# sdwyc/ROLO

Measured on AMD Instinct MI355X. Metric: scans/sec (128k-pt frame, 20 GN iters), higher is better.
Workload: dtype f64

## Files before the change

rolo_amd/csrc/knn_cov.hip:

```cpp
#include <cstdio>
#include <cstring>
#include <string.h>
#include "rolo_internal.hpp"
#include "switches.hpp"
#include "dev_math.hpp"
#include "voxel_dev.hpp"
#ifdef ROLO_KNN_ROCPRIM_SORT
#include <rocprim/rocprim.hpp>
#endif
#include <cfloat>
#include <climits>

namespace rolo {

namespace {


constexpr int BBOX_BLOCKS = 128;
constexpr int BBOX_PART = 16;

__global__ __launch_bounds__(256) void bbox_kernel(KnnPair A, int* bbox) {
  __shared__ float smn[4][3], smx[4][3];
  const int which = blockIdx.x / BBOX_BLOCKS, blk = blockIdx.x - which * BBOX_BLOCKS;
  const float4* __restrict__ p = A.c[which].xyz;
// ... 512 lines not shown
bool knn_voxel_fuse_supported() {
#ifdef ROLO_KNN_ROCPRIM_SORT
  return false;
#else
  return true;
#endif
}

size_t knn_bbox_ints() { return BBOX_PART + 2 * BBOX_BLOCKS * 6; }

size_t knn_sort_temp_bytes(int n) {
#ifdef ROLO_KNN_ROCPRIM_SORT
  size_t bytes = 0;
  (void)rocprim::radix_sort_pairs(nullptr, bytes, (uint32_t*)nullptr, (uint32_t*)nullptr, (uint32_t*)nullptr, (uint32_t*)nullptr,
                                  (size_t)n, 0, 31, (hipStream_t)0);
  return bytes;
#else
  (void)n;
  return sizeof(int) * SORT_PASSES * SORT_NB * SORT_D;
#endif
}

hipError_t launch_knn_build(const KnnPair& A_in, void* sort_tmp, size_t sort_tmp_bytes, uint32_t* keys0, uint32_t* keys1,
                            uint32_t* vals0, uint32_t* vals1, int* bbox, const VoxelFuse& vf, hipStream_t s) {
  KnnPair A = A_in;
  bool have_parts = true;
  for (int i = 0; i < A.n_clouds; i++) have_parts = have_parts && A.c[i].bpart != nullptr && A.c[i].n_bpart > 0;
  if (!have_parts) for (int i = 0; i < A.n_clouds; i++) { A.c[i].bpart = bbox + BBOX_PART + i * BBOX_BLOCKS * 6; A.c[i].n_bpart = BBOX_BLOCKS; }
  const int nc = A.n_clouds;
  const int n_total = A.c[0].n + (nc > 1 ? A.c[1].n : 0);
#ifdef ROLO_KNN_ROCPRIM_SORT
  const int tile_ = ((n_total + SORT_NB - 1) / SORT_NB + SORT_T - 1) / SORT_T * SORT_T;
  if (!have_parts) bbox_kernel<<<BBOX_BLOCKS * nc, 256, 0, s>>>(A, bbox);
  morton_kernel<<<SORT_NB + (vf.enabled ? VF_CLEAR_BLOCKS : 0), SORT_T, 0, s>>>(A, bbox, keys0, vals0, n_total, tile_, nullptr, vf);
  hipError_t e = rocprim::radix_sort_pairs(sort_tmp, sort_tmp_bytes, keys0, keys1, vals0, vals1, (size_t)n_total, 0, nc > 1 ? KEY_BITS : KEY_BITS - 1, s);
  if (e != hipSuccess) return e;
  const uint32_t* order = vals1;
#else
  (void)sort_tmp_bytes;
  int* cnt = static_cast<int*>(sort_tmp);
  const int gvf = vf.enabled ? ((vf.n_tgt + SORT_PASSES - 1) / SORT_PASSES + SORT_T - 1) / SORT_T : 0;
  const int tile = ((n_total + SORT_NB - 1) / SORT_NB + SORT_T - 1) / SORT_T * SORT_T;
  if (!have_parts) bbox_kernel<<<BBOX_BLOCKS * nc, 256, 0, s>>>(A, bbox);
  morton_kernel<<<SORT_NB + (vf.enabled ? VF_CLEAR_BLOCKS : 0), SORT_T, 0, s>>>(A, bbox, keys0, vals0, n_total, tile, cnt, vf);
  uint32_t *ki = keys0, *vi = vals0, *ko = keys1, *vo = vals1;
  for (int p = 0; p < SORT_PASSES; p++) {
    if (p > 0) sort_hist_kernel<<<SORT_NB, SORT_T, 0, s>>>(ki, n_total, tile, p, cnt);
    sort_scatter_kernel<<<SORT_NB + gvf, SORT_T, 0, s>>>(ki, vi, ko, vo, n_total, tile, p, cnt, vf);
    uint32_t* t1 = ki; ki = ko; ko = t1; t1 = vi; vi = vo; vo = t1;
  }
  const uint32_t* order = vi;
#endif
  static_assert(256 % KNN_LEAF == 0 && (KNN_LEAF & (KNN_LEAF - 1)) == 0, "leaf_kernel reduces a leaf inside a wavefront");
  const int l0 = (A.c[0].P * KNN_LEAF + 255) / 256, l1 = nc > 1 ? (A.c[1].P * KNN_LEAF + 255) / 256 : 0;
  leaf_kernel<<<l0 + l1, 256, 0, s>>>(A, l0, order);
  constexpr int LPB = 256 / KNN_LEAF;
  int count0 = A.c[0].P >= LPB ? A.c[0].P / LPB : A.c[0].P, count1 = nc > 1 ? (A.c[1].P >= LPB ? A.c[1].P / LPB : A.c[1].P) : 1;
  while (count0 > 1 || count1 > 1) {
    const int chunk0 = count0 < 512 ? count0 : 512, chunk1 = count1 < 512 ? count1 : 512;
    const int b0 = count0 > 1 ? count0 / chunk0 : 0, b1 = count1 > 1 ? count1 / chunk1 : 0;
    tree_reduce_kernel<<<b0 + b1, 256, 0, s>>>(A.c[0].boxes, count0, chunk0, b0, nc > 1 ? A.c[1].boxes : nullptr, count1, chunk1);
    if (count0 > 1) count0 /= chunk0;
    if (count1 > 1) count1 /= chunk1;
  }
  return hipGetLastError();
}

#ifdef ROLO_KNN_STATS
extern "C" int rolo_debug_wave_records(unsigned* out ) {
  (void)hipDeviceSynchronize();
  return hipMemcpyFromSymbol(out, HIP_SYMBOL(g_knn_wave_rec), sizeof(unsigned) * 16384 * 8) == hipSuccess ? 0 : -1;
}
#endif

static inline int slice_blocks(const KnnCloud& c) { return (c.q_end - c.q_begin + 255) / 256; }

constexpr int KNN_SUB_MAX_PACKETS = 1792;
hipError_t launch_knn_walk(const KnnPair& A, int k, hipStream_t s, int* lanes_out, bool device_busy, bool moments) {
  if (lanes_out) *lanes_out = 1;
  constexpr int QPB = 256;
  const int n0 = A.c[0].q_end - A.c[0].q_begin, n1 = A.n_clouds > 1 ? A.c[1].q_end - A.c[1].q_begin : 0;
  const int g0 = (n0 + QPB - 1) / QPB, g1 = (n1 + QPB - 1) / QPB;
  if (g0 + g1 == 0) return hipSuccess;
  if (k > 64) {
    KnnPair R = A;
    for (int r = 0; 64 * r < k; r++) {
      const int kr = k - 64 * r < 64 ? k - 64 * r : 64;
      for (int i = 0; i < R.n_clouds; i++) { R.c[i].slot0 = 64 * r; R.c[i].k_total = k; }
      if (r == 0) knn_walk_kernel<64><<<g0 + g1, 256, 0, s>>>(R, g0, kr);
      else knn_walk_kernel<64, true><<<g0 + g1, 256, 0, s>>>(R, g0, kr);
    }
    return hipGetLastError();
  }
  if (k == 20) {
    const int sub_env = switches().knn_sub;
    const int packets = (n0 + 63) / 64 + (n1 + 63) / 64;
    const int lanes = sub_env < 0 ? (packets <= KNN_SUB_MAX_PACKETS ? 4 : (device_busy ? 0 : 2)) : (sub_env == 2 ? 2 : (sub_env ? 4 : 0));
    if (lanes_out) *lanes_out = lanes ? lanes : 1;
    if (lanes == 4) { const int s0 = (n0 + 63) / 64, s1 = (n1 + 63) / 64; if (moments) knn_walk_sub_kernel<4, true><<<s0 + s1, 256, 0, s>>>(A, s0); else knn_walk_sub_kernel<4><<<s0 + s1, 256, 0, s>>>(A, s0); }
    else if (lanes == 2) { const int s0 = (n0 + 127) / 128, s1 = (n1 + 127) / 128; if (moments) knn_walk_sub_kernel<2, true><<<s0 + s1, 256, 0, s>>>(A, s0); else knn_walk_sub_kernel<2><<<s0 + s1, 256, 0, s>>>(A, s0); }
    else if (moments) knn_walk_kernel<20, false, true><<<g0 + g1, 256, 0, s>>>(A, g0, k);
    else knn_walk_kernel<20><<<g0 + g1, 256, 0, s>>>(A, g0, k);
  }
  else if (k > 32) knn_walk_kernel<64><<<g0 + g1, 256, 0, s>>>(A, g0, k);
  else knn_walk_kernel<32><<<g0 + g1, 256, 0, s>>>(A, g0, k);
  return hipGetLastError();
}

hipError_t launch_knn_unstage(const KnnPair& A, bool own_slice_only, const VoxelFuse& vf, hipStream_t s) {
  const int g0 = own_slice_only ? slice_blocks(A.c[0]) : (A.c[0].n_sorted + 255) / 256;
  const int g1 = A.n_clouds > 1 ? (own_slice_only ? slice_blocks(A.c[1]) : (A.c[1].n_sorted + 255) / 256) : 0;
  if (g0 + g1 == 0) return hipSuccess;
  VoxelFuse v = vf;
  if (own_slice_only) v.enabled = 0;
  knn_unstage_kernel<<<g0 + g1, 256, 0, s>>>(A, g0, own_slice_only ? 1 : 0, v);
  return hipGetLastError();
}

hipError_t launch_knn_tail(const KnnPair& A, int k, int regularization, const VoxelFuse& vf, hipStream_t s, bool moments) {
  const int g0 = slice_blocks(A.c[0]), g1 = A.n_clouds > 1 ? slice_blocks(A.c[1]) : 0;
  if (g0 + g1 == 0) return hipSuccess;
  if (k > 64) knn_tail_loop_kernel<<<g0 + g1, 256, 0, s>>>(A, g0, k, regularization, vf);
  else if (k == 20 && moments) knn_tail_kernel<20, true><<<g0 + g1, 256, 0, s>>>(A, g0, k, regularization, vf);
  else if (k == 20) knn_tail_kernel<20><<<g0 + g1, 256, 0, s>>>(A, g0, k, regularization, vf);
  else if (k <= 32) knn_tail_kernel<32><<<g0 + g1, 256, 0, s>>>(A, g0, k, regularization, vf);
  else knn_tail_kernel<64><<<g0 + g1, 256, 0, s>>>(A, g0, k, regularization, vf);
  return hipGetLastError();
}

}
```

rolo_amd/csrc/knn_packet.hpp:

```cpp
#pragma once
#include "rolo_internal.hpp"
#include "dev_math.hpp"
#include "knn_seed_net.hpp"
#include <cfloat>
#include <climits>

#ifndef KNN_STAT
#ifdef ROLO_KNN_STATS
#define KNN_STAT(x) x
#else
#define KNN_STAT(x)
#endif
#endif

namespace rolo {
namespace {

constexpr int WALK_STACK = KNN_WALK_STACK;

ROLO_DEV float box_d2(const float4& lo, const float4& hi, const float4& q) {
  float dx = fmaxf(fmaxf(__fsub_rn(lo.x, q.x), __fsub_rn(q.x, hi.x)), 0.f);
  float dy = fmaxf(fmaxf(__fsub_rn(lo.y, q.y), __fsub_rn(q.y, hi.y)), 0.f);
  float dz = fmaxf(fmaxf(__fsub_rn(lo.z, q.z), __fsub_rn(q.z, hi.z)), 0.f);
  return __fadd_rn(__fadd_rn(__fmul_rn(dx, dx), __fmul_rn(dy, dy)), __fmul_rn(dz, dz));
}

ROLO_DEV double key_pack(float d2, int idx) {
  return __longlong_as_double((long long)(((unsigned long long)__float_as_uint(d2) << 32) | (unsigned)idx));
}
ROLO_DEV float key_d2(double k) { return __uint_as_float((unsigned)((unsigned long long)__double_as_longlong(k) >> 32)); }
ROLO_DEV int key_idx(double k) { return (int)(unsigned)((unsigned long long)__double_as_longlong(k) & 0xffffffffull); }

ROLO_DEV double vmin_f64(double a, double b) { double r; asm("v_min_f64 %0, %1, %2" : "=v"(r) : "v"(a), "v"(b)); return r; }
ROLO_DEV double vmax_f64(double a, double b) { double r; asm("v_max_f64 %0, %1, %2" : "=v"(r) : "v"(a), "v"(b)); return r; }
#ifndef ROLO_KNN_SPLIT_MINMAX
ROLO_DEV void insert_slot(double& ks, double ksm1, double c) { asm("v_min_f64 %0, %1, %0\n\tv_max_f64 %0, %2, %0" : "+&v"(ks) : "v"(c), "v"(ksm1)); }
#else
ROLO_DEV void insert_slot(double& ks, double ksm1, double c) { ks = vmax_f64(ksm1, vmin_f64(c, ks)); }
#endif
#ifndef ROLO_KNN_B1
#define ROLO_KNN_B1 15
#define ROLO_KNN_B2 10
#define ROLO_KNN_B3 5
#endif
template <int KMAX>
ROLO_DEV void insert_tiered(double (&K)[KMAX], double ck) {
  constexpr int B1 = KMAX == 20 ? ROLO_KNN_B1 : 3 * (KMAX / 4), B2 = KMAX == 20 ? ROLO_KNN_B2 : 2 * (KMAX / 4), B3 = KMAX == 20 ? ROLO_KNN_B3 : KMAX / 4;
#pragma unroll
  for (int s = KMAX - 1; s >= B1; s--) insert_slot(K[s], K[s - 1], ck);
  if (__any(ck < K[B1 - 1])) {
#pragma unroll
    for (int s = B1 - 1; s >= B2; s--) insert_slot(K[s], K[s - 1], ck);
    if (__any(ck < K[B2 - 1])) {
#pragma unroll
      for (int s = B2 - 1; s >= B3; s--) insert_slot(K[s], K[s - 1], ck);
      if (__any(ck < K[B3 - 1])) {
#pragma unroll
        for (int s = B3 - 1; s >= 1; s--) insert_slot(K[s], K[s - 1], ck);
        K[0] = vmin_f64(ck, K[0]);
      }
    }
  }
}

ROLO_DEV void sload_leaf(const float4* __restrict__ p, float4 (&pts)[KNN_LEAF]) {
#pragma unroll
  for (int u = 0; u < KNN_LEAF; u++) pts[u] = p[u];
}
ROLO_DEV void sload_node(const float4* __restrict__ p, float4& llo, float4& lhi, float4& rlo, float4& rhi) { llo = p[0]; lhi = p[1]; rlo = p[2]; rhi = p[3]; }

template <int KMAX, bool LOWER = false>
ROLO_DEV void knn_score_leaf(const float4* __restrict__ sorted, int g, const float4& q, double (&K)[KMAX], int kk, double& bkey, float& bd,
                             unsigned& n_ins, unsigned& lane_acc, unsigned& rounds, double lo = 0.0) {
  float4 pts[KNN_LEAF];
  sload_leaf(sorted + KNN_LEAF * (size_t)g, pts);
  KNN_STAT(const double bkey0 = bkey; unsigned my_acc = 0;)
#ifdef ROLO_KNN_STATS2
  unsigned my_cur = 0;
#endif
#pragma unroll
  for (int u = 0; u < KNN_LEAF; u++) {
    const float4 c = pts[u];
    const float dx = q.x - c.x, dy = q.y - c.y, dz = q.z - c.z;
    const float cd = ((dx * dx) + (dy * dy)) + (dz * dz);
    const double ck0 = key_pack(cd, __float_as_int(c.w));
    const double ck = (LOWER && !(ck0 > lo)) ? key_pack(INFINITY, INT_MAX) : ck0;
    KNN_STAT(if (__any(ck < bkey)) { n_ins++; lane_acc += (unsigned)__popcll(__ballot(ck < bkey)); })
    KNN_STAT(if (ck < bkey0) my_acc++;)
#ifdef ROLO_KNN_STATS2
    if (ck < bkey) my_cur++;
#endif
    if (ck < bkey) {
      insert_tiered<KMAX>(K, ck);
#pragma unroll
      for (int s = 0; s < KMAX; s++) if (s == kk - 1) bkey = K[s];
      bd = key_d2(bkey);
    }
  }
#ifdef ROLO_KNN_STATS
#ifdef ROLO_KNN_STATS2
  rounds += my_cur;
  (void)my_acc;
#else
  { unsigned m = my_acc;
    for (int off = 32; off > 0; off >>= 1) m = max(m, (unsigned)__shfl_xor((int)m, off, 64));
    rounds += m; }
#endif
#endif
}

struct KeyMin { ROLO_DEV double operator()(double a, double b) const { return vmin_f64(a, b); } };
struct KeyMax { ROLO_DEV double operator()(double a, double b) const { return vmax_f64(a, b); } };

template <int NB, int STRIDE, class P>
ROLO_DEV void seed_chunk(const P& p, int first, const float4& q, double (&K)[20]) {
  double b[NB];
#pragma unroll
  for (int u = 0; u < NB; u++) {
    const float4 c = p[first + u * STRIDE];
    const float dx = q.x - c.x, dy = q.y - c.y, dz = q.z - c.z;
    const float cd = ((dx * dx) + (dy * dy)) + (dz * dz);
    b[u] = key_pack(cd, __float_as_int(c.w));
  }
  if constexpr (NB == 8) seednet::sort8(b, KeyMin(), KeyMax()); else seednet::sort4(b, KeyMin(), KeyMax());
  seednet::merge_chunk<NB>(K, b, KeyMin(), KeyMax());
}

ROLO_DEV void knn_seed_leaf(const float4* __restrict__ sorted, int g, const float4& q, double (&K)[20]) {
  static_assert(KNN_LEAF == 16, "two chunks of 8");
  float4 pts[KNN_LEAF];
  sload_leaf(sorted + KNN_LEAF * (size_t)g, pts);
  seed_chunk<8, 1>(pts, 0, q, K);
  seed_chunk<8, 1>(pts, 8, q, K);
}

template <int CTRL>
ROLO_DEV double dpp_f64(double x) {
  const long long v = __double_as_longlong(x);
  const int lo = __builtin_amdgcn_mov_dpp((int)(unsigned)(unsigned long long)v, CTRL, 0xF, 0xF, true);
  const int hi = __builtin_amdgcn_mov_dpp((int)(unsigned)((unsigned long long)v >> 32), CTRL, 0xF, 0xF, true);
  return __longlong_as_double((long long)(((unsigned long long)(unsigned)hi << 32) | (unsigned)lo));
}
template <int ST> ROLO_DEV double sub_xchg(double x) { return ST == 0 ? dpp_f64<0xB1>(x) : ST == 1 ? dpp_f64<0x4E>(x) : dpp_f64<0x141>(x); }
template <int SUB> ROLO_DEV double sub_min(double x) {
  x = vmin_f64(x, sub_xchg<0>(x));
  if (SUB >= 4) x = vmin_f64(x, sub_xchg<1>(x));
  if (SUB >= 8) x = vmin_f64(x, sub_xchg<2>(x));
  return x;
}
template <int SUB> ROLO_DEV double sub_max(double x) {
  x = vmax_f64(x, sub_xchg<0>(x));
  if (SUB >= 4) x = vmax_f64(x, sub_xchg<1>(x));
  if (SUB >= 8) x = vmax_f64(x, sub_xchg<2>(x));
  return x;
}

ROLO_DEV int xcd_contiguous_block(int b, int G, int wpb = 4) {
#ifdef ROLO_KNN_NO_XCD_REMAP
  return b;
#else
  if (G * wpb <= 2048) {
    const int x = b & 7, k = b >> 3, q = G >> 3, r = G & 7;
    return x * q + min(x, r) + k;
  }
  const int RUN = 256 / wpb, GROUP = 8 * RUN;
  if (b >= G / GROUP * GROUP) return b;
  const int grp = b / GROUP, o = b - grp * GROUP;
  return grp * GROUP + (o & 7) * RUN + (o >> 3);
#endif
}

typedef __attribute__((address_space(3))) int lds_int;

template <int KMAX, bool LOWER>
ROLO_DEV void packet_walk(const float4* __restrict__ sorted, const float4* __restrict__ boxes, int P, int g_own0, int g_own1, const float4& q, double (&K)[KMAX], int kk,
                          double& bkey, float& bd, double lo, lds_int* stk, int& sp, int h,
                          unsigned& st_nodes, unsigned& st_leaves, unsigned& st_ins, unsigned& st_lane, unsigned& st_rounds, unsigned& st_push) {
  (void)st_push;
  while (true) {
    h = __builtin_amdgcn_readfirstlane(h);
    if (h < P) {
      st_nodes++;
      float4 llo, lhi, rlo, rhi;
      sload_node(boxes + 4 * (size_t)h, llo, lhi, rlo, rhi);
      const float bl = box_d2(llo, lhi, q), br = box_d2(rlo, rhi, q);
      const bool okl = (bl <= bd) && (bl < INFINITY), okr = (br <= bd) && (br < INFINITY);
      const unsigned long long ml = __ballot(okl), mr = __ballot(okr);
      if (ml != 0ull && mr != 0ull) {
        const unsigned long long pref = __ballot((okl || okr) && (bl <= br));
        const bool left_first = 2 * __popcll(pref) >= __popcll(ml | mr);
        if (sp < WALK_STACK) { stk[sp] = left_first ? 2 * h + 1 : 2 * h; sp++; KNN_STAT(st_push++;) }
        h = left_first ? 2 * h : 2 * h + 1;
        continue;
      }
      if (ml != 0ull) { h = 2 * h; continue; }
      if (mr != 0ull) { h = 2 * h + 1; continue; }
    } else {
      const int g = h - P;
      if (g < g_own0 || g >= g_own1) {
        knn_score_leaf<KMAX, LOWER>(sorted, g, q, K, kk, bkey, bd, st_ins, st_lane, st_rounds, lo);
        st_leaves++;
      }
    }
    if (sp == 0) return;
    sp--;
    h = stk[sp];
  }
}

}
}
```

rolo_amd/csrc/knn_walk.hpp:

```cpp
#pragma once
#ifdef ROLO_KNN_STATS
#define KNN_STAT(x) x
#else
#define KNN_STAT(x)
#endif
#include "knn_packet.hpp"

namespace rolo {
namespace {

ROLO_DEV double* stage_area(const KnnCloud& cl, unsigned add) {
  double* s = cl.stage;
  if (cl.stage_epoch) {
    const unsigned long long e = __hip_atomic_load(cl.stage_epoch, __ATOMIC_RELAXED, __HIP_MEMORY_SCOPE_SYSTEM) + add;
    if (e & 1ull) s += cl.stage_alt;
  }
  return s;
}

#ifdef ROLO_KNN_STATS
__device__ unsigned g_knn_wave_rec[16384][8];
#endif

template <int KMAX>
ROLO_DEV void walk_write_lists(const KnnCloud& cl, const double (&K)[KMAX], int kk, double bkey, int qi, int j) {
  int ki[KMAX];
#pragma unroll
  for (int u = 0; u < KMAX; u++) ki[u] = key_idx(K[u]);
  const int slot0 = (KMAX == 64) ? cl.slot0 : 0;
  const int ktot = (KMAX == 64 && cl.k_total) ? cl.k_total : kk;
  if (cl.knn_idx) {
#pragma unroll
    for (int u = 0; u < KMAX; u++) if (u < kk) { cl.knn_idx[(size_t)qi * ktot + slot0 + u] = ki[u]; cl.knn_d2[(size_t)qi * ktot + slot0 + u] = key_d2(K[u]); }
  }
  if (KMAX == 64 && cl.lower) cl.lower[j] = bkey;
  int32_t* __restrict__ nbr = cl.nbr;
#pragma unroll
  for (int u = 0; u < KMAX; u++) nbr[(size_t)(slot0 + u) * cl.n_sorted + j] = ki[u];
}

template <int KMAX>
ROLO_DEV void walk_write_moments(const KnnCloud& cl, const double (&K)[KMAX], int kk, int qi, int j, int (*s_ki)[256]) {
  if (cl.knn_idx) {
#pragma unroll
    for (int u = 0; u < KMAX; u++) if (u < kk) { cl.knn_idx[(size_t)qi * kk + u] = key_idx(K[u]); cl.knn_d2[(size_t)qi * kk + u] = key_d2(K[u]); }
  }
  const int tid = threadIdx.x;
#pragma unroll
  for (int u = 0; u < KMAX; u++) s_ki[u][tid] = key_idx(K[u]);
  const float4* __restrict__ orig = cl.xyz;
  double mx = 0, my = 0, mz = 0;
#pragma unroll 5
  for (int u = 0; u < kk; u++) { const float4 p = orig[s_ki[u][tid]]; mx += (double)p.x; my += (double)p.y; mz += (double)p.z; }
  mx /= kk; my /= kk; mz /= kk;
  double cxx = 0, cxy = 0, cxz = 0, cyy = 0, cyz = 0, czz = 0;
#pragma unroll 5
  for (int u = 0; u < kk; u++) {
    const float4 p = orig[s_ki[u][tid]];
    const double ax = (double)p.x - mx, ay = (double)p.y - my, az = (double)p.z - mz;
    cxx += ax * ax; cxy += ax * ay; cxz += ax * az; cyy += ay * ay; cyz += ay * az; czz += az * az;
  }
  double* __restrict__ mom = reinterpret_cast<double*>(cl.nbr);
  const size_t pitch = (size_t)cl.n_sorted;
  mom[j] = cxx / kk; mom[pitch + j] = cxy / kk; mom[2 * pitch + j] = cxz / kk; mom[3 * pitch + j] = cyy / kk; mom[4 * pitch + j] = cyz / kk; mom[5 * pitch + j] = czz / kk;
}

#ifndef ROLO_KNN_WALK_OCC
#define ROLO_KNN_WALK_OCC 4
#endif
#ifndef ROLO_KNN_PACKET
#define ROLO_KNN_PACKET 64
#endif
#ifndef ROLO_KNN_SEED_EXTRA
#define ROLO_KNN_SEED_EXTRA 1
#endif
static_assert(ROLO_KNN_PACKET == 64, "one query per lane");

template <int KMAX, bool LOWER>
ROLO_DEV void walk_seeds(const float4* __restrict__ sorted, int g_mine0, int g_own0, int g_own1, int n_leaves, const float4& q, bool active, double (&K)[KMAX], int kk, double& bkey, float& bd, double lo,
                         unsigned& st_leaves, unsigned& st_ins, unsigned& st_lane, unsigned& st_rounds) {
  const int n_own = min(g_mine0 + 64 / KNN_LEAF, n_leaves) - g_mine0, n_before = g_mine0 - g_own0;
  for (int i = 0; i < g_own1 - g_own0; i++) {
    const int g = i < n_own ? g_mine0 + i : (i - n_own < n_before ? g_own0 + (i - n_own) : g_mine0 + (i - n_before));
    if constexpr (KMAX == 20 && !LOWER) knn_seed_leaf(sorted, g, q, K);
    else knn_score_leaf<KMAX, LOWER>(sorted, g, q, K, kk, bkey, bd, st_ins, st_lane, st_rounds, lo);
    st_leaves++;
  }
  if constexpr (KMAX == 20 && !LOWER) {
    if (active) { bkey = K[KMAX - 1]; bd = key_d2(bkey); }
  }
}

template <int KMAX, bool LOWER = false, bool MOMENTS = false>
__global__ __launch_bounds__(256, KMAX > 32 ? 2 : (MOMENTS ? 6 : ROLO_KNN_WALK_OCC)) void knn_walk_kernel(KnnPair A, int split, int k) {
  __shared__ int stk[4][WALK_STACK];
  __shared__ int s_ki[MOMENTS ? KMAX : 1][256];
  const int tid = threadIdx.x;
  const int wv = tid >> 6;
  const int blk = xcd_contiguous_block((int)blockIdx.x, (int)gridDim.x, 4);
  const int which = blk >= split ? 1 : 0;
  const float4* __restrict__ sorted = A.c[which].sorted;
  const float4* __restrict__ boxes = A.c[which].boxes;
  const int n_sorted = A.c[which].n_sorted, P = A.c[which].P;
  const int lane_ = tid & 63;
  const int j = A.c[which].q_begin + (blk - (which ? split : 0)) * 256 + wv * 64 + lane_;
  float4 q = make_float4(0.f, 0.f, 0.f, 0.f);
  int qi = INT_MAX;
  if (j < A.c[which].q_end) { q = sorted[j]; qi = __float_as_int(q.w); }
  const bool active = qi != INT_MAX;
  const int kk = (KMAX == 20) ? 20 : k;
  const int n_leaves = n_sorted / KNN_LEAF;
  unsigned st_nodes = 0, st_leaves = 0, st_ins = 0, st_lane = 0, st_rounds = 0, st_push = 0;

  const double sentinel = key_pack(INFINITY, INT_MAX);
  double K[KMAX];
#pragma unroll
  for (int u = 0; u < KMAX; u++) K[u] = sentinel;
  float bd = active ? INFINITY : -1.0f;
  double bkey = active ? sentinel : key_pack(0.f, 0);

  const int g_mine0 = __builtin_amdgcn_readfirstlane(j / KNN_LEAF);
  const int g_own0 = max(g_mine0 - ROLO_KNN_SEED_EXTRA, 0);
  const int g_own1 = min(g_mine0 + 64 / KNN_LEAF + ROLO_KNN_SEED_EXTRA, n_leaves);
  double lo = 0.0;
  if (LOWER && active) lo = A.c[which].lower[j];
  (void)lo;
  walk_seeds<KMAX, LOWER>(sorted, g_mine0, g_own0, g_own1, n_leaves, q, active, K, kk, bkey, bd, lo, st_leaves, st_ins, st_lane, st_rounds);

  int sp = 0;
  int h = 1;
#ifdef ROLO_KNN_STATS
  unsigned long long wt0;
  asm("s_memrealtime %0\n\ts_waitcnt lgkmcnt(0)\n\ts_mov_b32 %1, 1" : "=s"(wt0), "=s"(h));
#endif
  packet_walk<KMAX, LOWER>(sorted, boxes, P, g_own0, g_own1, q, K, kk, bkey, bd, lo, (lds_int*)&stk[wv][0], sp, h, st_nodes, st_leaves, st_ins, st_lane, st_rounds, st_push);
#ifdef ROLO_KNN_STATS
  { unsigned long long wt1; asm volatile("s_memrealtime %0\n\ts_waitcnt lgkmcnt(0)" : "=s"(wt1));
    unsigned st_rounds_rec = st_rounds;
#ifdef ROLO_KNN_STATS2
    for (int off = 32; off > 0; off >>= 1) st_rounds_rec = max(st_rounds_rec, (unsigned)__shfl_xor((int)st_rounds_rec, off, 64));
#endif
    const unsigned wid = blockIdx.x * 4 + (threadIdx.x >> 6);
    if ((threadIdx.x & 63) == 0 && wid < 16384) {
      g_knn_wave_rec[wid][0] = st_nodes; g_knn_wave_rec[wid][1] = st_leaves; g_knn_wave_rec[wid][2] = st_ins; g_knn_wave_rec[wid][3] = st_push;
      g_knn_wave_rec[wid][4] = (unsigned)wt0; g_knn_wave_rec[wid][5] = (unsigned)wt1; g_knn_wave_rec[wid][6] = st_lane; g_knn_wave_rec[wid][7] = st_rounds_rec;
    } }
#endif
  (void)st_nodes; (void)st_leaves; (void)st_ins; (void)st_lane; (void)st_rounds; (void)st_push;

  if (!active) return;

  if (MOMENTS) {
    walk_write_moments<KMAX>(A.c[which], K, kk, qi, j, s_ki);
    return;
  }
  walk_write_lists<KMAX>(A.c[which], K, kk, bkey, qi, j);
}

template <int ST> ROLO_DEV void merge20(double (&K)[20]) {
#pragma unroll
  for (int j = 0; j < 10; j++) {
    const double o1 = sub_xchg<ST>(K[19 - j]), o2 = sub_xchg<ST>(K[j]);
    K[j] = vmin_f64(K[j], o1);
    K[19 - j] = vmin_f64(K[19 - j], o2);
  }
  seednet::bitonic_clean<20, 0, false>(K, KeyMin(), KeyMax());
}

template <int SUB, bool MOMENTS = false>
__global__ __launch_bounds__(256, MOMENTS ? 6 : ROLO_KNN_WALK_OCC) void knn_walk_sub_kernel(KnnPair A, int split ) {
  constexpr int SH = SUB == 2 ? 1 : 2, QPW = 64 / SUB, PPL = KNN_LEAF / SUB, KMAX = 20, E = 4 / SUB , OWN = QPW / KNN_LEAF;
  static_assert(SUB == 2 || SUB == 4, "lanes per query");
  static_assert(KNN_LEAF == 16, "a wavefront's queries are whole leaves");
  __shared__ int stk_[4][WALK_STACK];
  __shared__ int s_ki[MOMENTS ? KMAX : 1][256];
  const int tid = threadIdx.x;
  const int wv = __builtin_amdgcn_readfirstlane(tid >> 6), lane = tid & 63, sub = lane & (SUB - 1), ql = lane >> SH;
  const int blk = xcd_contiguous_block((int)blockIdx.x, (int)gridDim.x, 4);
  const int which = blk >= split ? 1 : 0;
  const KnnCloud& cl = A.c[which];
  const float4* __restrict__ sorted = cl.sorted;
  const float4* __restrict__ boxes = cl.boxes;
  const int n_sorted = cl.n_sorted, P = cl.P, n_leaves = n_sorted / KNN_LEAF;
  const int j0 = cl.q_begin + ((blk - (which ? split : 0)) * 4 + wv) * QPW;
  const int j = j0 + ql;
  float4 q = make_float4(0.f, 0.f, 0.f, 0.f);
  int qi = INT_MAX;
  if (j < cl.q_end) { q = sorted[j]; qi = __float_as_int(q.w); }
  const bool active = qi != INT_MAX;
  const double sentinel = key_pack(INFINITY, INT_MAX);
  double K[KMAX];
#pragma unroll
  for (int u = 0; u < KMAX; u++) K[u] = sentinel;
  double B = active ? sentinel : key_pack(0.f, 0);
  float bd = active ? INFINITY : -1.0f;
  auto score = [&](int g) {
    const float4* __restrict__ leaf = sorted + KNN_LEAF * (size_t)g;
    bool changed = false;
#pragma unroll
    for (int t0 = 0; t0 < PPL; t0 += 4) {
      float4 c[4];
#pragma unroll
      for (int t = 0; t < 4; t++) c[t] = leaf[(t0 + t) * SUB + sub];
#pragma unroll
      for (int t = 0; t < 4; t++) {
        const float dx = q.x - c[t].x, dy = q.y - c[t].y, dz = q.z - c[t].z;
        const float cd = ((dx * dx) + (dy * dy)) + (dz * dz);
        const double ck = key_pack(cd, __float_as_int(c[t].w));
        if (ck < B) { insert_tiered<KMAX>(K, ck); changed = true; }
      }
    }
    if (__any(changed)) {
      B = vmin_f64(vmin_f64(B, sub_min<SUB>(K[KMAX - 1])), sub_max<SUB>(K[KMAX / SUB - 1]));
      bd = key_d2(B);
    }
  };
  const int g_mine = min(j0 / KNN_LEAF, n_leaves - 1);
  const int g_own0 = max(g_mine - ROLO_KNN_SEED_EXTRA, 0), g_own1 = min(g_mine + OWN + ROLO_KNN_SEED_EXTRA, n_leaves);
// ... 199 lines not shown
```

rolo_amd/csrc/loopicp.hip:

```cpp
#include "keymap.hpp"
#include "knn_packet.hpp"
#include <cfloat>
#include <climits>
#include <cmath>
#include <cstring>
#include <vector>

namespace rolo {
int ctx_build_map_trees(rolo_ctx* c, const float* corner, int nc, const float* surf, int ns, int stride, KnnPair* out, bool on_device = false);
void** ctx_loop_slot(rolo_ctx* c);
hipStream_t ctx_stream(rolo_ctx* c);
int ctx_device(rolo_ctx* c);

namespace {

constexpr int ICP_THREADS = 256;
constexpr int ICP_NV = 17;

struct IcpArgs {
  const float4* cur;
  int n_sorted;
  const float4* tsorted;
  const float4* tboxes;
  const float4* txyz;
  int P, n_leaves;
  float cap2;
  double* partials;
  int32_t* idx_out;
  float* d2_out;
};

ROLO_DEV unsigned long long icp_key(float d2, int idx) { return ((unsigned long long)__float_as_uint(d2) << 32) | (unsigned)idx; }

__global__ __launch_bounds__(ICP_THREADS) void icp_assoc_kernel(IcpArgs A) {
  __shared__ int stk_[ICP_THREADS / 64][WALK_STACK];
  __shared__ double red[ICP_THREADS / 64][ICP_NV];
  const int wv = __builtin_amdgcn_readfirstlane(threadIdx.x >> 6), lane = threadIdx.x & 63;
  const int j = blockIdx.x * ICP_THREADS + threadIdx.x;
  float4 qs = make_float4(0.f, 0.f, 0.f, __int_as_float(INT_MAX));
  if (j < A.n_sorted) qs = A.cur[j];
  const int qidx = __float_as_int(qs.w);
  const bool active = qidx != INT_MAX;
  const float4 q = make_float4(active ? qs.x : 0.f, active ? qs.y : 0.f, active ? qs.z : 0.f, 0.f);
  unsigned long long best = active ? icp_key(A.cap2, INT_MAX) : 0ull;
  float bd = active ? A.cap2 : -1.0f;
  {
    const float4* __restrict__ sorted = A.tsorted;
    const float4* __restrict__ boxes = A.tboxes;
    const int P = A.P, n_leaves = A.n_leaves;
    lds_int* stk = (lds_int*)&stk_[wv][0];
    int sp = 0, h = 1;
    while (true) {
      h = __builtin_amdgcn_readfirstlane(h);
      if (h < P) {
        float4 llo, lhi, rlo, rhi;
        sload_node(boxes + 4 * (size_t)h, llo, lhi, rlo, rhi);
        const float bl = box_d2(llo, lhi, q), br = box_d2(rlo, rhi, q);
        const bool okl = (bl <= bd) && (bl < INFINITY), okr = (br <= bd) && (br < INFINITY);
        const unsigned long long ml = __ballot(okl), mr = __ballot(okr);
        if (ml != 0ull && mr != 0ull) {
          const unsigned long long pref = __ballot((okl || okr) && (bl <= br));
          const bool left_first = 2 * __popcll(pref) >= __popcll(ml | mr);
          if (sp < WALK_STACK) { stk[sp] = left_first ? 2 * h + 1 : 2 * h; sp++; }
          h = left_first ? 2 * h : 2 * h + 1;
          continue;
        }
        if (ml != 0ull) { h = 2 * h; continue; }
        if (mr != 0ull) { h = 2 * h + 1; continue; }
      } else if (h - P < n_leaves) {
        float4 pts[KNN_LEAF];
        sload_leaf(sorted + KNN_LEAF * (size_t)(h - P), pts);
#pragma unroll
        for (int u = 0; u < KNN_LEAF; u++) {
          const float4 c = pts[u];
          const float dx = q.x - c.x, dy = q.y - c.y, dz = q.z - c.z;
          const float cd = ((dx * dx) + (dy * dy)) + (dz * dz);
          const unsigned long long ck = icp_key(cd, __float_as_int(c.w));
          best = ck < best ? ck : best;
        }
        bd = active ? __uint_as_float((unsigned)(best >> 32)) : -1.0f;
      }
      if (sp == 0) break;
      sp--;
      h = stk[sp];
    }
  }
  const int ti = (int)(unsigned)(best & 0xffffffffull);
  const bool kept = active && ti != INT_MAX;
  const float d2 = __uint_as_float((unsigned)(best >> 32));
  double acc[ICP_NV];
#pragma unroll
  for (int v = 0; v < ICP_NV; v++) acc[v] = 0.0;
  if (kept) {
    const float4 t = A.txyz[ti];
    const double p[3] = {(double)qs.x, (double)qs.y, (double)qs.z}, qq[3] = {(double)t.x, (double)t.y, (double)t.z};
    acc[0] = 1.0; acc[1] = (double)d2;
#pragma unroll
    for (int r = 0; r < 3; r++) {
      acc[2 + r] = p[r]; acc[5 + r] = qq[r];
#pragma unroll
      for (int c = 0; c < 3; c++) acc[8 + 3 * r + c] = p[r] * qq[c];
    }
  }
  if (active && A.idx_out) { A.idx_out[qidx] = kept ? ti : -1; A.d2_out[qidx] = kept ? d2 : INFINITY; }
#pragma unroll
  for (int v = 0; v < ICP_NV; v++) {
    double x = acc[v];
#pragma unroll
    for (int off = 32; off > 0; off >>= 1) x += __shfl_xor(x, off, 64);
    if (lane == 0) red[wv][v] = x;
  }
  __syncthreads();
  if (threadIdx.x < ICP_NV) {
    double s = 0;
#pragma unroll
    for (int w = 0; w < ICP_THREADS / 64; w++) s += red[w][threadIdx.x];
    A.partials[(size_t)blockIdx.x * ICP_NV + threadIdx.x] = s;
  }
}

__global__ __launch_bounds__(256) void icp_sum_kernel(const double* __restrict__ partials, int nblocks, double* __restrict__ out) {
  __shared__ double part[8][32];
  const int v = threadIdx.x & 31, q = threadIdx.x >> 5;
  double s = 0;
  if (v < ICP_NV) for (int b = q; b < nblocks; b += 8) s += partials[(size_t)b * ICP_NV + v];
  part[q][v] = s;
  __syncthreads();
  if (threadIdx.x < ICP_NV) {
    double t = 0;
#pragma unroll
    for (int k = 0; k < 8; k++) t += part[k][threadIdx.x];
    out[threadIdx.x] = t;
  }
}

struct Rows12 { float T[12]; };
template <bool KEEP_PAD>
__global__ __launch_bounds__(256) void icp_transform_kernel(const float4* in, float4* out , int n, Rows12 R) {
  const int i = blockIdx.x * 256 + threadIdx.x;
  if (i >= n) return;
// ... 367 lines not shown
```

rolo_amd/csrc/scan2map.hip:

```cpp
#include "rolo_internal.hpp"
#include "switches.hpp"
#include "dev_math.hpp"
#include "knn_packet.hpp"
#include <cfloat>
#include <climits>
#include <cmath>
#include <cstdio>
#include <cstring>
#include <vector>

namespace rolo {
int ctx_build_map_trees(rolo_ctx* c, const float* corner, int nc, const float* surf, int ns, int stride, KnnPair* out, bool on_device = false);
int keymap_device_submap(rolo_keymap* km, const float** d_corner, int* m_corner, const float** d_surf, int* m_surf, hipEvent_t* ready, hipEvent_t* consumed, int* device);
void keymap_mark_consumed(rolo_keymap* km);
extern "C" int rolo_ctx_acquire(int device, rolo_ctx** out);
extern "C" void rolo_ctx_release(rolo_ctx* c);
hipStream_t ctx_stream(rolo_ctx* c);
int ctx_device(rolo_ctx* c);
void ctx_set_error(const char* msg);

namespace {

constexpr int S2M_THREADS = 128;
constexpr int S2M_STACK = 40;
// ... 331 lines not shown
#pragma unroll
  for (int u = 0; u < 5; u++) o[u] = sub_xchg<ST>(K[u]);
#pragma unroll
  for (int u = 0; u < 5; u++) insert5(K, o[u]);
}

__global__ __launch_bounds__(256) void s2m_assoc_kernel(S2mArgs A, int split ) {
  constexpr int SUB = S2M_SUB, PPL = KNN_LEAF / SUB;
  static_assert(SUB == 4, "the two-level step tests one grandchild per sub-lane");
  __shared__ int stk_[4][WALK_STACK];
  __shared__ double red[4][S2M_NV];
  const int wv = __builtin_amdgcn_readfirstlane(threadIdx.x >> 6), lane = threadIdx.x & 63, sub = lane & (SUB - 1), ql = lane >> 2;
  const int blk = xcd_contiguous_block((int)blockIdx.x, (int)gridDim.x, 4);
  const bool corner = blk < split;
  const KnnCloud& Q = A.qry[corner ? 0 : 1];
  const KnnCloud& M = A.map[corner ? 0 : 1];
  const int j = ((blk - (corner ? 0 : split)) * 4 + wv) * S2M_FPW + ql;
  double acc[S2M_NV];
#pragma unroll
  for (int v = 0; v < S2M_NV; v++) acc[v] = 0.0;
  float4 qs = make_float4(0.f, 0.f, 0.f, __int_as_float(INT_MAX));
  if (j < Q.n_sorted) qs = Q.sorted[j];
  const int qidx = __float_as_int(qs.w);
  const bool active = qidx != INT_MAX;
  float sx, sy, sz;
  pointAssociateToMap(A.T, qs, sx, sy, sz);
  const float4 q = make_float4(active ? sx : 0.f, active ? sy : 0.f, active ? sz : 0.f, 0.f);
  const double sentinel = key_pack(INFINITY, INT_MAX);
  double K[5] = {sentinel, sentinel, sentinel, sentinel, sentinel};
  double B = active ? key_pack(1.0f, 0) : key_pack(0.f, 0);
  float bd = active ? 1.0f : -1.0f;
  int n_nodes = 0, n_leaves = 0;
  const long long t_walk0 = A.wstats ? wall_clock64() : 0;
  {
    const float4* __restrict__ sorted = M.sorted;
    const float4* __restrict__ boxes = M.boxes;
    const int P = M.P;
    lds_int* stk = (lds_int*)&stk_[wv][0];
    int sp = 0, h = 1;
    auto score = [&](const float4 (&c)[PPL]) {
      bool changed = false;
#pragma unroll
      for (int t = 0; t < PPL; t++) {
        const float dx = q.x - c[t].x, dy = q.y - c[t].y, dz = q.z - c[t].z;
        const float cd = ((dx * dx) + (dy * dy)) + (dz * dz);
        const double ck = key_pack(cd, __float_as_int(c[t].w));
        if (ck < B) { insert5(K, ck); changed = true; }
      }
      if (__any(changed)) {
        B = vmin_f64(vmin_f64(B, sub_min<SUB>(K[4])), vmax_f64(sub_max<SUB>(K[0]), sub_min<SUB>(K[1])));
        bd = key_d2(B);
      }
    };
    while (true) {
      h = __builtin_amdgcn_readfirstlane(h);
      if (2 * h < P) {
        n_nodes++;
        const float4 blo = boxes[8 * (size_t)h + 2 * sub], bhi = boxes[8 * (size_t)h + 2 * sub + 1];
        const float d = box_d2(blo, bhi, q);
        const bool ok = (d <= bd) && (d < INFINITY);
        const unsigned long long m = __ballot(ok);
        float dm = ok ? d : INFINITY;
        dm = fminf(dm, __int_as_float(__builtin_amdgcn_mov_dpp(__float_as_int(dm), 0xB1, 0xF, 0xF, true)));
        dm = fminf(dm, __int_as_float(__builtin_amdgcn_mov_dpp(__float_as_int(dm), 0x4E, 0xF, 0xF, true)));
        const unsigned long long v = __ballot(ok && d == dm);
        int key[4];
#pragma unroll
        for (int c = 0; c < 4; c++) {
          const unsigned long long sel = 0x1111111111111111ull << c;
          key[c] = (m & sel) != 0ull ? __popcll(v & sel) * 4 + (3 - c) : -1;
        }
        auto cx = [](int& a, int& bb) { const int hi = max(a, bb), lo = min(a, bb); a = hi; bb = lo; };
        cx(key[0], key[1]); cx(key[2], key[3]); cx(key[0], key[2]); cx(key[1], key[3]); cx(key[1], key[2]);
        if (key[0] >= 0) {
#pragma unroll
          for (int r = 3; r >= 1; r--) if (key[r] >= 0 && sp < WALK_STACK) { stk[sp] = 4 * h + (3 - (key[r] & 3)); sp++; }
          h = 4 * h + (3 - (key[0] & 3));
          continue;
        }
      } else if (h < P) {
        n_nodes++;
        float4 llo, lhi, rlo, rhi;
        sload_node(boxes + 4 * (size_t)h, llo, lhi, rlo, rhi);
        const float bl = box_d2(llo, lhi, q), br = box_d2(rlo, rhi, q);
        const bool okl = (bl <= bd) && (bl < INFINITY), okr = (br <= bd) && (br < INFINITY);
        const unsigned long long ml = __ballot(okl), mr = __ballot(okr);
        if (ml != 0ull && mr != 0ull) {
          const unsigned long long pref = __ballot((okl || okr) && (bl <= br));
          const bool left_first = 2 * __popcll(pref) >= __popcll(ml | mr);
          if (sp < WALK_STACK) { stk[sp] = left_first ? 2 * h + 1 : 2 * h; sp++; }
          h = left_first ? 2 * h : 2 * h + 1;
          continue;
        }
        if (ml != 0ull) { h = 2 * h; continue; }
        if (mr != 0ull) { h = 2 * h + 1; continue; }
      } else {
        const float4* __restrict__ leaf = sorted + KNN_LEAF * (size_t)(h - P);
        float4 c[PPL];
#pragma unroll
        for (int t = 0; t < PPL; t++) c[t] = leaf[t * SUB + sub];
        score(c);
        n_leaves++;
      }
      if (sp == 0) break;
      sp--;
      h = stk[sp];
    }
  }
  if (A.wstats && lane == 0) A.wstats[blk * 4 + wv] = make_int4(n_nodes, n_leaves, (int)(wall_clock64() - t_walk0), blk);
  merge5<0>(K);
  merge5<1>(K);
  if (active && sub == 0) {
    float bdv[5]; int bi[5];
#pragma unroll
    for (int u = 0; u < 5; u++) { bdv[u] = key_d2(K[u]); bi[u] = key_idx(K[u]); }
    s2m_feature(A, corner, M, qs, sx, sy, sz, bdv, bi, (corner ? 0 : A.n_corner) + qidx, acc);
  }
  s2m_block_sum<4>(acc, red, A.partials, blk);
}

__global__ __launch_bounds__(256) void s2m_sum_kernel(const double* __restrict__ partials, int nblocks, double* __restrict__ out) {
  __shared__ double part[8][32];
  const int v = threadIdx.x & 31, q = threadIdx.x >> 5;
  double s = 0;
  if (v < S2M_NV) {
    for (int b0 = q; b0 < nblocks; b0 += 64) {
      double r[8];
#pragma unroll
      for (int u = 0; u < 8; u++) { const int b = b0 + 8 * u; const double x = partials[(size_t)min(b, nblocks - 1) * S2M_NV + v]; r[u] = b < nblocks ? x : 0.0; }
#pragma unroll
      for (int u = 0; u < 8; u++) s += r[u];
    }
  }
  part[q][v] = s;
  __syncthreads();
  if (threadIdx.x < S2M_NV) {
    double t = 0;
#pragma unroll
    for (int k = 0; k < 8; k++) t += part[k][threadIdx.x];
    out[threadIdx.x] = t;
  }
}

bool solve_qr6f(const float* Ain, const float* bin, float* x) {
  float A[36], b[6];
  std::memcpy(A, Ain, sizeof(A)); std::memcpy(b, bin, sizeof(b));
  for (int k = 0; k < 6; k++) {
    float nrm = 0; for (int i = k; i < 6; i++) nrm += A[i * 6 + k] * A[i * 6 + k];
    nrm = std::sqrt(nrm);
    if (nrm == 0.f) return false;
    const float alpha = A[k * 6 + k] > 0 ? -nrm : nrm;
    float v[6] = {0, 0, 0, 0, 0, 0};
    for (int i = k; i < 6; i++) v[i] = A[i * 6 + k];
    v[k] -= alpha;
    float vv = 0; for (int i = k; i < 6; i++) vv += v[i] * v[i];
    if (vv == 0.f) continue;
    for (int j = k; j < 6; j++) { float d = 0; for (int i = k; i < 6; i++) d += v[i] * A[i * 6 + j]; d = 2 * d / vv; for (int i = k; i < 6; i++) A[i * 6 + j] -= d * v[i]; }
    { float d = 0; for (int i = k; i < 6; i++) d += v[i] * b[i]; d = 2 * d / vv; for (int i = k; i < 6; i++) b[i] -= d * v[i]; }
  }
  for (int i = 5; i >= 0; i--) {
    float s = b[i];
    for (int j = i + 1; j < 6; j++) s -= A[i * 6 + j] * x[j];
    if (A[i * 6 + i] == 0.f) return false;
    x[i] = s / A[i * 6 + i];
  }
  return true;
}
// ... 206 lines not shown
```

Before: 4474.

## Climb KNN tree from own leaf, pack box distances, read bound from list tail

```diff
diff --git a/rolo_amd/csrc/knn_box_pair.hpp b/rolo_amd/csrc/knn_box_pair.hpp
--- /dev/null
+++ b/rolo_amd/csrc/knn_box_pair.hpp
@@ -0,0 +1,51 @@
+#pragma once
+#include <cfloat>
+#include <cmath>
+
+#if defined(__HIPCC__) || defined(__CUDACC__)
+#define ROLO_BOX_FN __host__ __device__ __forceinline__
+#else
+#define ROLO_BOX_FN inline
+#endif
+
+namespace rolo {
+
+#if defined(__clang__)
+typedef float box_f2 __attribute__((ext_vector_type(2)));
+#else
+typedef float box_f2 __attribute__((vector_size(8)));
+#endif
+
+template <class V4>
+ROLO_BOX_FN float box_d2(const V4& lo, const V4& hi, const V4& q) {
+  const float dx = fmaxf(fmaxf(lo.x - q.x, q.x - hi.x), 0.f);
+  const float dy = fmaxf(fmaxf(lo.y - q.y, q.y - hi.y), 0.f);
+  const float dz = fmaxf(fmaxf(lo.z - q.z, q.z - hi.z), 0.f);
+  return ((dx * dx) + (dy * dy)) + (dz * dz);
+}
+
+template <class V4>
+ROLO_BOX_FN box_f2 box_d2_pair(const V4& llo, const V4& lhi, const V4& rlo, const V4& rhi, const V4& q) {
+  const box_f2 qx = {q.x, q.x}, qy = {q.y, q.y}, qz = {q.z, q.z};
+  const box_f2 lox = {llo.x, rlo.x}, loy = {llo.y, rlo.y}, loz = {llo.z, rlo.z};
+  const box_f2 hix = {lhi.x, rhi.x}, hiy = {lhi.y, rhi.y}, hiz = {lhi.z, rhi.z};
+  const box_f2 ax = lox - qx, bx = qx - hix, ay = loy - qy, by = qy - hiy, az = loz - qz, bz = qz - hiz;
+  const box_f2 dx = {fmaxf(fmaxf(ax[0], bx[0]), 0.f), fmaxf(fmaxf(ax[1], bx[1]), 0.f)};
+  const box_f2 dy = {fmaxf(fmaxf(ay[0], by[0]), 0.f), fmaxf(fmaxf(ay[1], by[1]), 0.f)};
+  const box_f2 dz = {fmaxf(fmaxf(az[0], bz[0]), 0.f), fmaxf(fmaxf(az[1], bz[1]), 0.f)};
+  return ((dx * dx) + (dy * dy)) + (dz * dz);
+}
+
+ROLO_BOX_FN float box_bound_clamp(float bd) {
+  int b, m;
+  const float fmax = FLT_MAX;
+  __builtin_memcpy(&b, &bd, 4); __builtin_memcpy(&m, &fmax, 4);
+  b = b < m ? b : m;
+  float r;
+  __builtin_memcpy(&r, &b, 4);
+  return r;
+}
+ROLO_BOX_FN bool box_reached(float d, float bd_clamped) { return d <= bd_clamped; }
+ROLO_BOX_FN bool box_reached_two_compares(float d, float bd) { return (d <= bd) && (d < INFINITY); }
+
+}
diff --git a/rolo_amd/csrc/knn_cov.hip b/rolo_amd/csrc/knn_cov.hip
--- a/rolo_amd/csrc/knn_cov.hip
+++ b/rolo_amd/csrc/knn_cov.hip
@@ -618,6 +618,7 @@
   const int n0 = A.c[0].q_end - A.c[0].q_begin, n1 = A.n_clouds > 1 ? A.c[1].q_end - A.c[1].q_begin : 0;
   const int g0 = (n0 + QPB - 1) / QPB, g1 = (n1 + QPB - 1) / QPB;
   if (g0 + g1 == 0) return hipSuccess;
+  for (int i = 0; i < A.n_clouds; i++) if (A.c[i].q_end > A.c[i].q_begin && A.c[i].q_begin % 64 != 0) return hipErrorInvalidValue;
   if (k > 64) {
     KnnPair R = A;
     for (int r = 0; 64 * r < k; r++) {
diff --git a/rolo_amd/csrc/knn_packet.hpp b/rolo_amd/csrc/knn_packet.hpp
--- a/rolo_amd/csrc/knn_packet.hpp
+++ b/rolo_amd/csrc/knn_packet.hpp
@@ -2,6 +2,7 @@
 #include "rolo_internal.hpp"
 #include "dev_math.hpp"
 #include "knn_seed_net.hpp"
+#include "knn_box_pair.hpp"
 #include <cfloat>
 #include <climits>
 
@@ -17,13 +18,6 @@
 namespace {
 
 constexpr int WALK_STACK = KNN_WALK_STACK;
-
-ROLO_DEV float box_d2(const float4& lo, const float4& hi, const float4& q) {
-  float dx = fmaxf(fmaxf(__fsub_rn(lo.x, q.x), __fsub_rn(q.x, hi.x)), 0.f);
-  float dy = fmaxf(fmaxf(__fsub_rn(lo.y, q.y), __fsub_rn(q.y, hi.y)), 0.f);
-  float dz = fmaxf(fmaxf(__fsub_rn(lo.z, q.z), __fsub_rn(q.z, hi.z)), 0.f);
-  return __fadd_rn(__fadd_rn(__fmul_rn(dx, dx), __fmul_rn(dy, dy)), __fmul_rn(dz, dz));
-}
 
 ROLO_DEV double key_pack(float d2, int idx) {
   return __longlong_as_double((long long)(((unsigned long long)__float_as_uint(d2) << 32) | (unsigned)idx));
@@ -68,13 +62,16 @@
   for (int u = 0; u < KNN_LEAF; u++) pts[u] = p[u];
 }
 ROLO_DEV void sload_node(const float4* __restrict__ p, float4& llo, float4& lhi, float4& rlo, float4& rhi) { llo = p[0]; lhi = p[1]; rlo = p[2]; rhi = p[3]; }
+
+template <int KMAX, bool LOWER> constexpr bool walk_bound_in_list() { return KMAX == 20 && !LOWER; }
 
 template <int KMAX, bool LOWER = false>
 ROLO_DEV void knn_score_leaf(const float4* __restrict__ sorted, int g, const float4& q, double (&K)[KMAX], int kk, double& bkey, float& bd,
                              unsigned& n_ins, unsigned& lane_acc, unsigned& rounds, double lo = 0.0) {
   float4 pts[KNN_LEAF];
   sload_leaf(sorted + KNN_LEAF * (size_t)g, pts);
-  KNN_STAT(const double bkey0 = bkey; unsigned my_acc = 0;)
+  constexpr bool IN_LIST = walk_bound_in_list<KMAX, LOWER>();
+  KNN_STAT(const double bkey0 = IN_LIST ? K[KMAX - 1] : bkey; unsigned my_acc = 0;)
 #ifdef ROLO_KNN_STATS2
   unsigned my_cur = 0;
 #endif
@@ -85,16 +82,19 @@
     const float cd = ((dx * dx) + (dy * dy)) + (dz * dz);
     const double ck0 = key_pack(cd, __float_as_int(c.w));
     const double ck = (LOWER && !(ck0 > lo)) ? key_pack(INFINITY, INT_MAX) : ck0;
-    KNN_STAT(if (__any(ck < bkey)) { n_ins++; lane_acc += (unsigned)__popcll(__ballot(ck < bkey)); })
+    const bool better = IN_LIST ? ck < K[KMAX - 1] : ck < bkey;
+    KNN_STAT(if (__any(better)) { n_ins++; lane_acc += (unsigned)__popcll(__ballot(better)); })
     KNN_STAT(if (ck < bkey0) my_acc++;)
 #ifdef ROLO_KNN_STATS2
-    if (ck < bkey) my_cur++;
-#endif
-    if (ck < bkey) {
+    if (better) my_cur++;
+#endif
+    if (better) {
       insert_tiered<KMAX>(K, ck);
-#pragma unroll
-      for (int s = 0; s < KMAX; s++) if (s == kk - 1) bkey = K[s];
-      bd = key_d2(bkey);
+      if constexpr (!IN_LIST) {
+#pragma unroll
+        for (int s = 0; s < KMAX; s++) if (s == kk - 1) bkey = K[s];
+        bd = key_d2(bkey);
+      }
     }
   }
 #ifdef ROLO_KNN_STATS
@@ -183,8 +183,9 @@
       st_nodes++;
       float4 llo, lhi, rlo, rhi;
       sload_node(boxes + 4 * (size_t)h, llo, lhi, rlo, rhi);
-      const float bl = box_d2(llo, lhi, q), br = box_d2(rlo, rhi, q);
-      const bool okl = (bl <= bd) && (bl < INFINITY), okr = (br <= bd) && (br < INFINITY);
+      const box_f2 d = box_d2_pair(llo, lhi, rlo, rhi, q);
+      const float bl = d[0], br = d[1], bdc = box_bound_clamp(walk_bound_in_list<KMAX, LOWER>() ? key_d2(K[KMAX - 1]) : bd);
+      const bool okl = box_reached(bl, bdc), okr = box_reached(br, bdc);
       const unsigned long long ml = __ballot(okl), mr = __ballot(okr);
       if (ml != 0ull && mr != 0ull) {
         const unsigned long long pref = __ballot((okl || okr) && (bl <= br));
@@ -208,5 +209,23 @@
   }
 }
 
-}
-}
+template <int KMAX, bool LOWER>
+ROLO_DEV void packet_climb(const float4* __restrict__ sorted, const float4* __restrict__ boxes, int P, int g_mine0, int g_own0, int g_own1, const float4& q, double (&K)[KMAX], int kk,
+                           double& bkey, float& bd, double lo, lds_int* stk,
+                           unsigned& st_nodes, unsigned& st_leaves, unsigned& st_ins, unsigned& st_lane, unsigned& st_rounds, unsigned& st_push) {
+  for (int a = (P + g_mine0) >> 2; a > 1; a >>= 1) {
+    const int s = a ^ 1;
+    const float4* __restrict__ rec = boxes + 4 * (size_t)(a >> 1) + 2 * (s & 1);
+    const float4 slo = rec[0], shi = rec[1];
+    const float d = box_d2(slo, shi, q);
+    const float bdc = box_bound_clamp(walk_bound_in_list<KMAX, LOWER>() ? key_d2(K[KMAX - 1]) : bd);
+    KNN_STAT(st_nodes++;)
+    if (__ballot(box_reached(d, bdc)) != 0ull) {
+      int sp = 0;
+      packet_walk<KMAX, LOWER>(sorted, boxes, P, g_own0, g_own1, q, K, kk, bkey, bd, lo, stk, sp, s, st_nodes, st_leaves, st_ins, st_lane, st_rounds, st_push);
+    }
+  }
+}
+
+}
+}
diff --git a/rolo_amd/csrc/knn_walk.hpp b/rolo_amd/csrc/knn_walk.hpp
--- a/rolo_amd/csrc/knn_walk.hpp
+++ b/rolo_amd/csrc/knn_walk.hpp
@@ -87,7 +87,10 @@
     st_leaves++;
   }
   if constexpr (KMAX == 20 && !LOWER) {
-    if (active) { bkey = K[KMAX - 1]; bd = key_d2(bkey); }
+    if (!active) {
+#pragma unroll
+      for (int u = 0; u < KMAX; u++) K[u] = key_pack(0.f, 0);
+    }
   }
 }
 
@@ -104,7 +107,7 @@
   const int n_sorted = A.c[which].n_sorted, P = A.c[which].P;
   const int lane_ = tid & 63;
   const int j = A.c[which].q_begin + (blk - (which ? split : 0)) * 256 + wv * 64 + lane_;
-  float4 q = make_float4(0.f, 0.f, 0.f, 0.f);
+  float4 q = make_float4(INFINITY, INFINITY, INFINITY, 0.f);
   int qi = INT_MAX;
   if (j < A.c[which].q_end) { q = sorted[j]; qi = __float_as_int(q.w); }
   const bool active = qi != INT_MAX;
@@ -127,13 +130,13 @@
   (void)lo;
   walk_seeds<KMAX, LOWER>(sorted, g_mine0, g_own0, g_own1, n_leaves, q, active, K, kk, bkey, bd, lo, st_leaves, st_ins, st_lane, st_rounds);
 
-  int sp = 0;
-  int h = 1;
+  int g_climb = g_mine0;
 #ifdef ROLO_KNN_STATS
   unsigned long long wt0;
-  asm("s_memrealtime %0\n\ts_waitcnt lgkmcnt(0)\n\ts_mov_b32 %1, 1" : "=s"(wt0), "=s"(h));
-#endif
-  packet_walk<KMAX, LOWER>(sorted, boxes, P, g_own0, g_own1, q, K, kk, bkey, bd, lo, (lds_int*)&stk[wv][0], sp, h, st_nodes, st_leaves, st_ins, st_lane, st_rounds, st_push);
+  { int zero; asm("s_memrealtime %0\n\ts_waitcnt lgkmcnt(0)\n\ts_mov_b32 %1, 0" : "=s"(wt0), "=s"(zero)); g_climb += zero; }
+#endif
+  if (g_mine0 < n_leaves)
+    packet_climb<KMAX, LOWER>(sorted, boxes, P, g_climb, g_own0, g_own1, q, K, kk, bkey, bd, lo, (lds_int*)&stk[wv][0], st_nodes, st_leaves, st_ins, st_lane, st_rounds, st_push);
 #ifdef ROLO_KNN_STATS
   { unsigned long long wt1; asm volatile("s_memrealtime %0\n\ts_waitcnt lgkmcnt(0)" : "=s"(wt1));
     unsigned st_rounds_rec = st_rounds;
diff --git a/rolo_amd/csrc/loopicp.hip b/rolo_amd/csrc/loopicp.hip
--- a/rolo_amd/csrc/loopicp.hip
+++ b/rolo_amd/csrc/loopicp.hip
@@ -55,7 +55,8 @@
       if (h < P) {
         float4 llo, lhi, rlo, rhi;
         sload_node(boxes + 4 * (size_t)h, llo, lhi, rlo, rhi);
-        const float bl = box_d2(llo, lhi, q), br = box_d2(rlo, rhi, q);
+        const box_f2 bd2 = box_d2_pair(llo, lhi, rlo, rhi, q);
+        const float bl = bd2[0], br = bd2[1];
         const bool okl = (bl <= bd) && (bl < INFINITY), okr = (br <= bd) && (br < INFINITY);
         const unsigned long long ml = __ballot(okl), mr = __ballot(okr);
         if (ml != 0ull && mr != 0ull) {
diff --git a/rolo_amd/csrc/scan2map.hip b/rolo_amd/csrc/scan2map.hip
--- a/rolo_amd/csrc/scan2map.hip
+++ b/rolo_amd/csrc/scan2map.hip
@@ -437,7 +437,8 @@
         n_nodes++;
         float4 llo, lhi, rlo, rhi;
         sload_node(boxes + 4 * (size_t)h, llo, lhi, rlo, rhi);
-        const float bl = box_d2(llo, lhi, q), br = box_d2(rlo, rhi, q);
+        const box_f2 bd2 = box_d2_pair(llo, lhi, rlo, rhi, q);
+        const float bl = bd2[0], br = bd2[1];
         const bool okl = (bl <= bd) && (bl < INFINITY), okr = (br <= bd) && (br < INFINITY);
         const unsigned long long ml = __ballot(okl), mr = __ballot(okr);
         if (ml != 0ull && mr != 0ull) {
```

Result: faster. 4661, median of 6 (+4.2%).
